# dansolombrino/Kindergarten-VQ-VAE

Measured on AMD Instinct MI355X. Metric: dSentences train sentences/sec, higher is better.
Workload: dtype bf16

## Files before the change

### include/kvq.h

```cpp
#ifndef KVQ_H
#define KVQ_H

#include <stddef.h>
#include <stdint.h>

#ifdef __cplusplus
extern "C" {
#endif

#define KVQ_VERSION 100

#define KVQ_F32 0
#define KVQ_BF16 1

#define KVQ_OK 0
#define KVQ_E_INVALID (-1)
#define KVQ_E_WORKSPACE (-2)
#define KVQ_E_LAUNCH (-3)
#define KVQ_E_NODEVICE (-4)

int kvq_version(void);
const char* kvq_last_error(void);

#define KVQ_GRAPH_NODE_KERNEL 0
// ... 129 lines not shown

size_t kvq_attn_probs_workspace_bytes(int B, int nh, int Sq, int Sk);
int kvq_attn_probs(const void* q, const void* k, const void* v, const int64_t* mask, const float* lse, int B, int nh, int Sq, int Sk,
                   int dh, int ldq, int ldk, int ldv, int causal, float scale, int io_dtype, float* probs, double* table, void* ws,
                   size_t ws_bytes, void* stream);

int kvq_attn_set_variant(int variant);

#define KVQ_GEMM_NT 0
#define KVQ_GEMM_NN 1
#define KVQ_GEMM_TN 2
#define KVQ_GEMM_TILE_128x192 0
#define KVQ_GEMM_TILE_128x256 1
#define KVQ_GEMM_TILE_256x192 2
#define KVQ_GEMM_TILE_256x256 3
#define KVQ_GEMM_TILE_64x128 4
#define KVQ_GEMM_TILE_128x192H 5
#define KVQ_GEMM_PERSISTENT 0x100
typedef struct kvq_gemm_problem {
    const void* A;
    const void* B;
    void* C;
    const void* bias;
    int M, N, K;
    int lda, ldb, ldc;
    int accumulate;
} kvq_gemm_problem;
int kvq_gemm_bf16(const void* A, const void* B, const void* bias, void* C, int M, int N, int K, int lda, int ldb, int ldc,
                  int layout, int tile, int accumulate, void* stream);
int kvq_gemm_any_bf16(const void* A, const void* B, const void* bias, void* C, int M, int N, int K, int lda, int ldb, int ldc,
                      int layout, int accumulate, void* stream);
int kvq_gemm_grouped_bf16(const kvq_gemm_problem* problems, int n_problems, int layout, int tile, void* stream);
int kvq_gemm_grouped_mixed_bf16(const kvq_gemm_problem* problems, const int* tiles, int n_problems, int layout, void* stream);
int kvq_gemm_bf16_dropres(const void* A, const void* B, const void* bias, const void* R, void* C, int M, int N, int K, int lda, int ldb,
                          int ldc, int tile, float p_drop, uint64_t seed, uint32_t site, void* stream);
int kvq_gemm_bf16_gelu(const void* A, const void* B, const void* bias, void* Hout, void* Aout, int M, int N, int K, int lda, int ldb,
                       int ldc, int tile, void* stream);
int64_t kvq_gemm_dgelu_partial_rows(int64_t M, int tile);
int kvq_gemm_bf16_dgelu(const void* A, const void* B, const void* H, void* C, float* part, size_t part_bytes, int M, int N, int K,
                        int lda, int ldb, int ldc, int tile, void* stream);

size_t kvq_gemm_ce_stats_bytes(int M, int N);
int kvq_gemm_bf16_ce(const void* A, const void* B, const void* bias, void* C, int M, int N, int K, int lda, int ldb, int ldc, int V,
                     float* stats, size_t stats_bytes, void* stream);

int kvq_fp8_quantize(const void* x_bf16, int64_t rows, int cols, int64_t ld, void* out_fp8, float* amax, float* scale, void* stream);
int kvq_fp8_state_floats(void);
int kvq_fp8_quantize_delayed(const void* x_bf16, int64_t rows, int cols, int64_t ld, void* out_fp8, float* state, void* stream);
int kvq_fp8_update_scales(float* state, int nsites, float headroom, void* stream);
int kvq_fp8_quantize_segments(const void* src_bf16, const int64_t* seg_off, const int64_t* seg_n, int nseg, int64_t max_seg_n,
                              void* dst_fp8, float* amax, float* scale, void* stream);
int kvq_fp8_quantize_segments_periodic(const void* src_bf16, const int64_t* seg_off, const int64_t* seg_n, int nseg, int64_t max_seg_n,
                                       void* dst_fp8, float* amax, float* scale, const void* step_count_u64, int period, void* stream);
int kvq_gemm_fp8_nt(const void* A8, const void* B8, const float* scale_a, const float* scale_b, const void* bias, void* C, int M, int N,
                    int K, int lda, int ldb, int ldc, void* stream);
int kvq_dropout_residual_ln_fwd_fp8(const void* y, const void* resid, const float* gamma, const float* beta, int64_t N, int H,
                                    float eps, float p_drop, uint64_t seed, uint32_t site, void* out, void* pre, float* mean, float* rstd,
                                    void* out_fp8, float* fp8_state, void* stream);
int kvq_attn_fwd_fp8_ok(int Sq, int Sk);
int kvq_attn_fwd_fp8(const void* q, const void* k, const void* v, const int64_t* mask, int B, int nh, int Sq, int Sk, int dh,
                     int ldq, int ldk, int ldv, int ldo, int causal, float scale, float p_drop, uint64_t seed, uint32_t site,
                     void* out, float* lse, void* out_fp8, int ld8, float* fp8_state, void* stream);
int kvq_gemm_fp8_nt_gelu(const void* A8, const void* B8, const float* scale_a, const float* scale_b, const void* bias, void* Hout, void* Aout,
                         void* Aout_fp8, int ld8, float* fp8_state, int M, int N, int K, int lda, int ldb, int ldc, void* stream);

#define KVQ_FP8_E4M3 0
// ... 99 lines not shown
```

### kindergarten-vq-vae_amd/csrc/kvq_gemm2.hip

```cpp
#include <limits.h>
#include <stdlib.h>

#include <atomic>
#include <type_traits>

#include "kvq_common.h"

namespace kvq {
namespace g2 {

typedef __bf16 bf16x8 __attribute__((ext_vector_type(8)));
typedef short s16x4 __attribute__((ext_vector_type(4)));
typedef __attribute__((address_space(1))) const void* gptr_t;
typedef __attribute__((address_space(3))) void* lptr_t;
typedef __attribute__((address_space(3))) s16x4* l4ptr_t;

constexpr int BK = 64;
constexpr int ROWB = 128;
constexpr int MAX_PROBLEMS = 16;

struct Problem {
    const unsigned short* A;
    const unsigned short* B;
    unsigned short* C;
// ... 1029 lines not shown
    if (P.p[0].M < C::BM || P.p[0].N < C::BN) return fail(KVQ_E_INVALID, "kvq_gemm (persistent): the matrix must hold one whole tile");
    constexpr int LDSP = C::NS * C::STAGE + 2 * BIAS_SLOT;
    static_assert(LDSP <= 160 * 1024, "LDS budget (persistent)");
    static std::atomic<bool> attr_done{false};
    if (!attr_done) {
        hipError_t e = hipFuncSetAttribute(reinterpret_cast<const void*>(&gemm3_kernel<C, EPI>), hipFuncAttributeMaxDynamicSharedMemorySize, LDSP);
        if (e != hipSuccess) return fail(KVQ_E_LAUNCH, "hipFuncSetAttribute(gemm3): %s", hipGetErrorString(e));
        attr_done = true;
    }
    const int grid = P.ntiles < persistent_grid() ? P.ntiles : persistent_grid();
    hipLaunchKernelGGL((gemm3_kernel<C, EPI>), dim3((unsigned)grid), dim3(C::THREADS), LDSP, st, P);
    return check_launch("gemm3_kernel");
}

template <template <bool, bool> class T>
static int launch_layout(int layout, const Params& P, hipStream_t st) {
    switch (layout) {
        case KVQ_GEMM_NT: return launch_cfg<T<true, true>>(P, st);
        case KVQ_GEMM_NN: return launch_cfg<T<true, false>>(P, st);
        case KVQ_GEMM_TN: return launch_cfg<T<false, false>>(P, st);
    }
    return fail(KVQ_E_INVALID, "kvq_gemm_bf16: unknown layout %d", layout);
}

static void tile_of(int tile, int& bm, int& bn) {
    switch (tile) {
        case KVQ_GEMM_TILE_128x256: bm = 128; bn = 256; break;
        case KVQ_GEMM_TILE_256x192: bm = 256; bn = 192; break;
        case KVQ_GEMM_TILE_256x256: bm = 256; bn = 256; break;
        case KVQ_GEMM_TILE_64x128: bm = 64; bn = 128; break;
        case KVQ_GEMM_TILE_128x192H: bm = 128; bn = 192; break;
        default: bm = 128; bn = 192; break;
    }
}

}
}

using namespace kvq;

static int build_params(const kvq_gemm_problem* probs, int nprob, int layout, int tile, g2::Params& P, const char* who) {
    KVQ_REQUIRE(probs && nprob >= 1 && nprob <= g2::MAX_PROBLEMS, "%s: 1..%d problems per launch", who, g2::MAX_PROBLEMS);
    KVQ_REQUIRE(layout == KVQ_GEMM_NT || layout == KVQ_GEMM_NN || layout == KVQ_GEMM_TN, "%s: unknown layout %d", who, layout);
    const bool persistent = (tile & KVQ_GEMM_PERSISTENT) != 0;
    tile &= ~KVQ_GEMM_PERSISTENT;
    KVQ_REQUIRE(tile >= KVQ_GEMM_TILE_128x192 && tile <= KVQ_GEMM_TILE_128x192H, "%s: unknown tile %d", who, tile);
    KVQ_REQUIRE(!(persistent && (tile == KVQ_GEMM_TILE_64x128 || tile == KVQ_GEMM_TILE_128x192H)), "%s: the four-wave tiles have no persistent form", who);
    int bm, bn;
    g2::tile_of(tile, bm, bn);
    (void)persistent;
    P.nprob = nprob;
    int t0 = 0;
    for (int i = 0; i < nprob; ++i) {
        const kvq_gemm_problem& q = probs[i];
        KVQ_REQUIRE(q.A && q.B && q.C && q.M > 0 && q.N > 0 && q.K > 0, "%s: problem %d: bad argument", who, i);
        KVQ_REQUIRE(q.K % g2::BK == 0, "%s: problem %d: K=%d must be a multiple of %d", who, i, q.K, g2::BK);
        KVQ_REQUIRE(q.M % 8 == 0 && q.N % 8 == 0 && q.lda % 8 == 0 && q.ldb % 8 == 0 && q.ldc % 8 == 0 && q.M >= 8 && q.N >= 8,
                    "%s: problem %d: M, N, lda, ldb, ldc must be multiples of 8", who, i);
        KVQ_REQUIRE((((uintptr_t)q.A | (uintptr_t)q.B | (uintptr_t)q.C) & 15) == 0 && (!q.bias || ((uintptr_t)q.bias & 7) == 0),
                    "%s: problem %d: operands must be 16-byte aligned", who, i);
        const int a_cols = layout == KVQ_GEMM_TN ? q.M : q.K, b_cols = layout == KVQ_GEMM_NT ? q.K : q.N;
        KVQ_REQUIRE(q.lda >= a_cols && q.ldb >= b_cols && q.ldc >= q.N, "%s: problem %d: leading dimension too small", who, i);
        g2::Problem& d = P.p[i];
        d.A = (const unsigned short*)q.A; d.B = (const unsigned short*)q.B; d.C = (unsigned short*)q.C; d.bias = (const unsigned short*)q.bias;
        d.M = q.M; d.N = q.N; d.K = q.K; d.lda = q.lda; d.ldb = q.ldb; d.ldc = q.ldc;
        d.tiles_m = (q.M + bm - 1) / bm; d.tiles_n = (q.N + bn - 1) / bn;
// ... 108 lines not shown
    if (nb)
        if (int rc = build_params(sorted, nb, layout, KVQ_GEMM_TILE_256x256, P, who)) return rc;
    const int nbig = P.ntiles;
    if (nprob > nb) {
        if (int rc = build_params(sorted + nb, nprob - nb, layout, KVQ_GEMM_TILE_128x256, S, who)) return rc;
        for (int i = nb; i < nprob; ++i) {
            P.p[i] = S.p[i - nb];
            P.p[i].tile0 += nbig;
        }
        for (int i = nprob; i < g2::MAX_PROBLEMS; ++i) P.p[i] = P.p[0];
        P.ntiles = nbig + S.ntiles;
    }
    P.nprob = nprob;
    typedef g2::Cfg256x256<false, false> CA;
    typedef g2::Cfg128x256<false, false> CB;
    constexpr int LDS = CA::LDS > CB::LDS ? CA::LDS : CB::LDS;
    static std::atomic<bool> attr_done{false};
    if (!attr_done) {
        hipError_t e = hipFuncSetAttribute(reinterpret_cast<const void*>(&g2::gemm2_mixed_kernel<CA, CB>), hipFuncAttributeMaxDynamicSharedMemorySize, LDS);
        if (e != hipSuccess) return fail(KVQ_E_LAUNCH, "hipFuncSetAttribute(gemm2_mixed): %s", hipGetErrorString(e));
        attr_done = true;
    }
    hipLaunchKernelGGL((g2::gemm2_mixed_kernel<CA, CB>), dim3((unsigned)P.ntiles), dim3(CA::THREADS), LDS, (hipStream_t)stream, P, nbig);
    return check_launch("gemm2_mixed_kernel");
}

int kvq_gemm_bf16(const void* A, const void* B, const void* bias, void* C, int M, int N, int K, int lda, int ldb, int ldc,
                  int layout, int tile, int accumulate, void* stream) {
    kvq_gemm_problem q;
    q.A = A; q.B = B; q.C = C; q.bias = bias; q.M = M; q.N = N; q.K = K; q.lda = lda; q.ldb = ldb; q.ldc = ldc; q.accumulate = accumulate;
    return kvq_gemm_grouped_bf16(&q, 1, layout, tile, stream);
}

int kvq_gemm_bf16_gelu(const void* A, const void* B, const void* bias, void* Hout, void* Aout, int M, int N, int K, int lda, int ldb,
                       int ldc, int tile, void* stream) {
    KVQ_REQUIRE(Aout && ((uintptr_t)Aout & 15) == 0, "kvq_gemm_bf16_gelu: null / misaligned second output");
    const int base = tile & ~KVQ_GEMM_PERSISTENT;
    KVQ_REQUIRE(base == KVQ_GEMM_TILE_256x192 || base == KVQ_GEMM_TILE_128x256, "kvq_gemm_bf16_gelu: tile must be 256x192 or 128x256");
    kvq_gemm_problem q;
    q.A = A; q.B = B; q.C = Hout; q.bias = bias; q.M = M; q.N = N; q.K = K; q.lda = lda; q.ldb = ldb; q.ldc = ldc; q.accumulate = 0;
    g2::Params P;
    if (int rc = build_params(&q, 1, KVQ_GEMM_NT, tile, P, "kvq_gemm_bf16_gelu")) return rc;
    for (int i = 0; i < g2::MAX_PROBLEMS; ++i) P.p[i].C2 = (unsigned short*)Aout;
    hipStream_t st = (hipStream_t)stream;
    if (tile & KVQ_GEMM_PERSISTENT) {
        if (base == KVQ_GEMM_TILE_256x192) return g2::launch_persistent<g2::Cfg256x192<true, true>, g2::EPI_GELU>(P, st);
        return g2::launch_persistent<g2::Cfg128x256<true, true>, g2::EPI_GELU>(P, st);
    }
    if (tile == KVQ_GEMM_TILE_256x192) return g2::launch_cfg<g2::Cfg256x192<true, true>, g2::EPI_GELU>(P, st);
    return g2::launch_cfg<g2::Cfg128x256<true, true>, g2::EPI_GELU>(P, st);
}

int kvq_gemm_bf16_dropres(const void* A, const void* B, const void* bias, const void* R, void* C, int M, int N, int K, int lda, int ldb,
                          int ldc, int tile, float p_drop, uint64_t seed, uint32_t site, void* stream) {
    KVQ_REQUIRE(R && ((uintptr_t)R & 15) == 0, "kvq_gemm_bf16_dropres: null / misaligned residual");
    KVQ_REQUIRE(p_drop >= 0.f && p_drop < 1.f, "kvq_gemm_bf16_dropres: p_drop out of range");
    KVQ_REQUIRE(tile == KVQ_GEMM_TILE_128x192 || tile == KVQ_GEMM_TILE_128x256 || tile == KVQ_GEMM_TILE_64x128,
                "kvq_gemm_bf16_dropres: tile must be 128x192, 128x256 or 64x128");
    kvq_gemm_problem q;
    q.A = A; q.B = B; q.C = C; q.bias = bias; q.M = M; q.N = N; q.K = K; q.lda = lda; q.ldb = ldb; q.ldc = ldc; q.accumulate = 0;
    g2::Params P;
    if (int rc = build_params(&q, 1, KVQ_GEMM_NT, tile, P, "kvq_gemm_bf16_dropres")) return rc;
    for (int i = 0; i < g2::MAX_PROBLEMS; ++i) {
        g2::Problem& d = P.p[i];
        d.H = (const unsigned short*)R; d.seed = seed; d.seed_off = seed_offset_ptr(); d.site = site; d.thresh = drop_threshold(p_drop);
        d.inv_keep = p_drop > 0.f ? 1.0f / (1.0f - p_drop) : 1.0f;
// ... 87 lines not shown
```

### kindergarten-vq-vae_amd/kvq/_ffi.py

```python
from __future__ import annotations

import ctypes as C
import os

_PKG = os.path.dirname(os.path.dirname(os.path.abspath(__file__)))
LIB_PATH = os.environ.get("KVQ_LIB_PATH") or os.path.join(_PKG, "lib", "libkvq.so")

KVQ_F32, KVQ_BF16 = 0, 1

_vp, _i64, _int, _f32, _sz = C.c_void_p, C.c_int64, C.c_int, C.c_float, C.c_size_t

KVQ_REDUCE_MAX_ITEMS = 32


class ReduceItem(C.Structure):
    _fields_ = [("src", _vp), ("dst", _vp), ("count", _i64), ("cols", _i64), ("ld", _i64), ("scale", _f32),
                ("src_dtype", C.c_int32), ("dst_dtype", C.c_int32), ("accumulate", C.c_int32)]


class GemmProblem(C.Structure):
    _fields_ = [("A", _vp), ("B", _vp), ("C", _vp), ("bias", _vp), ("M", _int), ("N", _int), ("K", _int),
                ("lda", _int), ("ldb", _int), ("ldc", _int), ("accumulate", _int)]


# ... 37 lines not shown
    "kvq_dropout_residual_ln_fwd": (_int, [_vp, _vp, _vp, _vp, _i64, _int, _f32, _f32, C.c_uint64, C.c_uint32, _int, _vp, _vp, _vp, _vp, _vp]),
    "kvq_ln_bwd_workspace_bytes": (_sz, [_i64, _int]),
    "kvq_dropout_residual_ln_bwd": (_int, [_vp, _vp, _vp, _vp, _vp, _i64, _int, _f32, C.c_uint64, C.c_uint32, _int, _vp, _vp, _vp, _vp, _vp,
                                           _int, _int, _vp, _sz, _vp]),
    "kvq_colsum_workspace_bytes": (_sz, [_i64, _i64]),
    "kvq_colsum": (_int, [_vp, _i64, _i64, _i64, _int, _vp, _int, _f32, _int, _vp, _sz, _vp]),
    "kvq_sum_slabs": (_int, [_vp, _int, _i64, _int, _vp, _vp]),
    "kvq_reduce_batch": (_int, [C.POINTER(ReduceItem), _int, _vp]),
    "kvq_ln_bwd_partial_rows": (_i64, [_i64]),
    "kvq_dropout_residual_ln_bwd_partial": (_int, [_vp, _vp, _vp, _vp, _vp, _i64, _int, _f32, C.c_uint64, C.c_uint32, _int, _vp, _vp,
                                                   _int, _vp, _sz, _vp]),
    "kvq_embed_ln_fwd": (_int, [_vp, _vp, _vp, _vp, _vp, _vp, _i64, _int, _int, _i64, _f32, _f32, C.c_uint64, C.c_uint32, _int, _vp, _vp,
                                _vp, _vp, _vp]),
    "kvq_ln_dropout_bwd_partial": (_int, [_vp, _vp, _vp, _vp, _vp, _i64, _int, _f32, C.c_uint64, C.c_uint32, _int, _vp, _vp, _sz, _vp]),
    "kvq_colsum_partial_rows": (_i64, [_i64]),
    "kvq_colsum_partial": (_int, [_vp, _i64, _i64, _i64, _int, _vp, _sz, _vp]),
    "kvq_gelu_fwd": (_int, [_vp, _vp, _i64, _int, _vp]),
    "kvq_gelu_bwd": (_int, [_vp, _vp, _vp, _i64, _int, _vp]),
    "kvq_gelu_bwd_partial_rows": (_i64, [_i64]),
    "kvq_gelu_bwd_bias": (_int, [_vp, _vp, _vp, _i64, _i64, _int, _vp, _sz, _vp]),
    "kvq_attn_fwd": (_int, [_vp, _vp, _vp, _vp, _int, _int, _int, _int, _int, _int, _int, _int, _int, _int, _f32, _f32,
                            C.c_uint64, C.c_uint32, _int, _vp, _vp, _vp]),
    "kvq_attn_bwd": (_int, [_vp, _vp, _vp, _vp, _vp, _int, _int, _int, _int, _int, _int, _int, _int, _int, _int, _f32, _f32,
                            C.c_uint64, C.c_uint32, _int, _vp, _vp, _vp, _vp, _vp, _vp, _int, _int, _vp]),
    "kvq_attn_bwd_saved": (_int, [_vp, _vp, _vp, _vp, _vp, _vp, _vp, _int, _int, _int, _int, _int, _int, _int, _int, _int, _int, _f32, _f32,
                                  C.c_uint64, C.c_uint32, _int, _vp, _vp, _vp, _vp, _vp, _vp, _int, _int, _vp]),
    "kvq_attn_probs_workspace_bytes": (_sz, [_int, _int, _int, _int]),
    "kvq_attn_probs": (_int, [_vp, _vp, _vp, _vp, _vp, _int, _int, _int, _int, _int, _int, _int, _int, _int, _f32, _int, _vp, _vp, _vp,
                              _sz, _vp]),
    "kvq_gemm_bf16": (_int, [_vp, _vp, _vp, _vp, _int, _int, _int, _int, _int, _int, _int, _int, _int, _vp]),
    "kvq_gemm_any_bf16": (_int, [_vp, _vp, _vp, _vp, _int, _int, _int, _int, _int, _int, _int, _int, _vp]),
    "kvq_gemm_grouped_bf16": (_int, [C.POINTER(GemmProblem), _int, _int, _int, _vp]),
    "kvq_gemm_grouped_mixed_bf16": (_int, [C.POINTER(GemmProblem), C.POINTER(_int), _int, _int, _vp]),
    "kvq_fp8_quantize": (_int, [_vp, _i64, _int, _i64, _vp, _vp, _vp, _vp]),
    "kvq_fp8_state_floats": (_int, []),
    "kvq_fp8_quantize_delayed": (_int, [_vp, _i64, _int, _i64, _vp, _vp, _vp]),
    "kvq_fp8_update_scales": (_int, [_vp, _int, _f32, _vp]),
    "kvq_fp8_quantize_segments": (_int, [_vp, _vp, _vp, _int, _i64, _vp, _vp, _vp, _vp]),
    "kvq_adam_step_dev_fp8": (_int, [_vp, _vp, _vp, _vp, _vp, _vp, _i64, _int, _vp, _f32, _f32, _f32, _f32, _f32, _vp, _vp, _vp, _vp, _vp, _int, _i64, _vp]),
    "kvq_fp8_quantize_segments_periodic": (_int, [_vp, _vp, _vp, _int, _i64, _vp, _vp, _vp, _vp, _int, _vp]),
    "kvq_gemm_fp8_nt": (_int, [_vp, _vp, _vp, _vp, _vp, _vp, _int, _int, _int, _int, _int, _int, _vp]),
    "kvq_gemm_fp8_nt_ex": (_int, [_vp, _vp, _vp, _vp, _vp, _vp, _int, _int, _int, _int, _int, _int, _int, _int, _vp]),
    "kvq_fp8_quantize_fmt": (_int, [_vp, _i64, _int, _i64, _vp, _vp, _vp, _int, _vp]),
    "kvq_fp8_quantize_delayed_fmt": (_int, [_vp, _i64, _int, _i64, _vp, _vp, _int, _vp]),
    "kvq_fp8_update_scales_fmt": (_int, [_vp, _int, _f32, _int, _vp]),
    "kvq_fp8_transpose": (_int, [_vp, _int, _int, _i64, _vp, _i64, _vp]),
    "kvq_fp8_transpose_segments": (_int, [_vp, _vp, _vp, _vp, _vp, _vp, _int, _i64, _vp]),
    "kvq_dropout_residual_ln_fwd_fp8": (_int, [_vp, _vp, _vp, _vp, _i64, _int, _f32, _f32, C.c_uint64, C.c_uint32, _vp, _vp, _vp, _vp, _vp, _vp, _vp]),
    "kvq_attn_fwd_fp8_ok": (_int, [_int, _int]),
    "kvq_attn_fwd_fp8": (_int, [_vp, _vp, _vp, _vp, _int, _int, _int, _int, _int, _int, _int, _int, _int, _int, _f32, _f32,
                                C.c_uint64, C.c_uint32, _vp, _vp, _vp, _int, _vp, _vp]),
    "kvq_gemm_fp8_nt_gelu": (_int, [_vp, _vp, _vp, _vp, _vp, _vp, _vp, _vp, _int, _vp, _int, _int, _int, _int, _int, _int, _vp]),
    "kvq_gemm_bf16_dropres": (_int, [_vp, _vp, _vp, _vp, _vp, _int, _int, _int, _int, _int, _int, _int, _f32, C.c_uint64, C.c_uint32, _vp]),
    "kvq_gemm_bf16_gelu": (_int, [_vp, _vp, _vp, _vp, _vp, _int, _int, _int, _int, _int, _int, _int, _vp]),
    "kvq_gemm_dgelu_partial_rows": (_i64, [_i64, _int]),
    "kvq_gemm_bf16_dgelu": (_int, [_vp, _vp, _vp, _vp, _vp, _sz, _int, _int, _int, _int, _int, _int, _int, _vp]),
    "kvq_attn_set_variant": (_int, [_int]),
    "kvq_adam_step": (_int, [_vp, _vp, _vp, _vp, _vp, _vp, _i64, _int, _f32, _f32, _f32, _f32, _f32, _i64, _f32, _vp]),
    "kvq_ce_forward_stats": (_int, [_vp, _vp, _i64, _i64, _int, _vp, _int, _vp, _vp, _vp, _vp, _vp, _vp]),
    "kvq_ce_forward_stats_ignore": (_int, [_vp, _vp, _i64, _i64, _int, _vp, _int, _i64, _vp, _vp, _vp, _vp, _vp, _vp, _vp]),
    "kvq_gemm_ce_stats_bytes": (_sz, [_int, _int]),
    "kvq_gemm_bf16_ce": (_int, [_vp, _vp, _vp, _vp, _int, _int, _int, _int, _int, _int, _int, _vp, _sz, _vp]),
    "kvq_step_state_advance": (_int, [_vp, _f32, _f32, C.POINTER(_i64), _int, _f32, _f32, _vp]),
    "kvq_adam_step_dev": (_int, [_vp, _vp, _vp, _vp, _vp, _vp, _i64, _int, _vp, _f32, _f32, _f32, _f32, _f32, _vp]),
    "kvq_set_seed_offset": (_int, [_vp]),
    "kvq_grad_sumsq_partials": (_int, []),
# ... 145 lines not shown
```

### kindergarten-vq-vae_amd/kvq/nnops.py

```python
from __future__ import annotations

import torch

from ._ffi import FP8_E4M3, FP8_E5M2, KvqError, check, io_dtype_of, lib, require_gpu, stream_ptr
from .functional import _workspace


def _p(t):
    return None if t is None else t.data_ptr()


def ln_fwd(y, resid, gamma, beta, eps, p_drop=0.0, seed=0, site=0, save_pre=True):
    require_gpu(y, gamma, beta)
    N, H = y.shape
    out = torch.empty_like(y)
    pre = torch.empty_like(y) if save_pre else None
    mean = torch.empty(N, dtype=torch.float32, device=y.device)
    rstd = torch.empty(N, dtype=torch.float32, device=y.device)
    check(lib().kvq_dropout_residual_ln_fwd(y.data_ptr(), _p(resid), gamma.data_ptr(), beta.data_ptr(), N, H, float(eps),
                                            float(p_drop), int(seed), int(site), io_dtype_of(y), out.data_ptr(), _p(pre),
                                            mean.data_ptr(), rstd.data_ptr(), stream_ptr()), "kvq_dropout_residual_ln_fwd")
    return out, pre, mean, rstd


def ln_fwd_fp8(y, resid, gamma, beta, eps, p_drop, seed, site, state, save_pre=True):
    require_gpu(y, gamma, beta)
    N, H = y.shape
    assert y.dtype == torch.bfloat16
    out = torch.empty_like(y)
    out8 = torch.empty((N, H), dtype=torch.uint8, device=y.device)
    pre = torch.empty_like(y) if save_pre else None
    mean = torch.empty(N, dtype=torch.float32, device=y.device)
    rstd = torch.empty(N, dtype=torch.float32, device=y.device)
# ... 455 lines not shown


def dropout(x, p_drop, seed, site, out=None):
    require_gpu(x)
    xc = x.contiguous()
    o = torch.empty_like(xc) if out is None else out
    check(lib().kvq_dropout(xc.data_ptr(), xc.numel(), float(p_drop), int(seed), int(site), io_dtype_of(xc), o.data_ptr(), stream_ptr()),
          "kvq_dropout")
    return o


def zero_ranges(tensors):
    import ctypes
    ts = [t for t in tensors if t is not None]
    if not ts:
        return
    ptrs = (ctypes.c_void_p * len(ts))(*[t.data_ptr() for t in ts])
    sizes = (ctypes.c_int64 * len(ts))(*[t.numel() * t.element_size() for t in ts])
    check(lib().kvq_zero_ranges(ptrs, sizes, len(ts), stream_ptr()), "kvq_zero_ranges")


def embed_grad(g, perm, sorted_ids, gW, accumulate=False):
    require_gpu(g, gW)
    N, H = g.shape
    l = lib()
    ws = _workspace(g.device, l.kvq_embed_grad_workspace_bytes(N, H), tag="embed_grad")
    check(l.kvq_embed_grad(g.data_ptr(), perm.data_ptr(), sorted_ids.data_ptr(), N, H, gW.shape[0], io_dtype_of(g), gW.data_ptr(),
                           io_dtype_of(gW), int(accumulate), ws.data_ptr(), ws.numel(), stream_ptr()), "kvq_embed_grad")
    return gW


_LAYOUTS = {"nt": 0, "nn": 1, "tn": 2}
TILES = {"128x192": 0, "128x256": 1, "256x192": 2, "256x256": 3, "64x128": 4, "128x192h": 5,
         "128x192p": 0x100, "128x256p": 0x101, "256x192p": 0x102, "256x256p": 0x103}
TILE_NAMES = {v: k for k, v in TILES.items()}
_TILE_DIMS = {0: (128, 192), 1: (128, 256), 2: (256, 192), 3: (256, 256), 4: (64, 128)}
def _gemm_dims(a, b, layout):
    if layout == "nt":
        (M, K), N = a.shape, b.shape[0]
    elif layout == "nn":
        (M, K), N = a.shape, b.shape[1]
    else:
        (K, M), N = a.shape, b.shape[1]
    return M, N, K


_TK_ALONE = {0: 0.459, 1: 0.557, 2: 0.891, 3: 1.035, 4: 0.296}
_TK_FULL = {0: 0.825, 1: 0.98, 2: 1.5, 3: 1.83, 4: 0.40}
_TK_PAIR = (0.45, 0.52)
_T_TILE = {0: 1.5, 1: 2.0, 2: 2.5, 3: 3.0, 4: 1.0}


def tile_cost_us(t, M, N, K, n_cu=256):
    bm, bn = _TILE_DIMS[t]
    n = -(-M // bm) * -(-N // bn)
    kt = max(K // 64, 1)
    f = min(n, n_cu) / n_cu
    lerp = lambda a, b: a + (b - a) * f
    w = -(-n // n_cu)
    if t == 4:
        return kt * ((w // 2) * lerp(*_TK_PAIR) + (w % 2) * lerp(_TK_ALONE[t], _TK_FULL[t])) + w * _T_TILE[t]
    return w * (kt * lerp(_TK_ALONE[t], _TK_FULL[t]) + _T_TILE[t])


def pick_tile(M, N, K=768, n_cu=256, candidates=None):
    cand = list(_TILE_DIMS) if candidates is None else [TILES[c] if isinstance(c, str) else c for c in candidates]
    return min(cand, key=lambda t: (tile_cost_us(t, M, N, K, n_cu), -_TILE_DIMS[t][0] * _TILE_DIMS[t][1]))


def persistent_pays(t, M, N, K, layout, accumulate=False, n_cu=256):
    bm, bn = _TILE_DIMS[t]
    if layout != "nt" or accumulate or t == 4 or M < bm or N < bn or K // 64 < 3:
        return False
    per_cu = -(-(-(-M // bm) * -(-N // bn)) // n_cu)
    return 3 <= per_cu <= 12


def cu_count(device):
    return torch.cuda.get_device_properties(device).multi_processor_count


def mixed_split(M, N, n_cu):
    tn = -(-N // 256)
    r = n_cu // tn * 256
    return r if 0 < r < M and -(-(M - r) // 128) * tn <= n_cu else 0

# ... 7 lines not shown


def gemm_problem(a, b, out, layout, bias=None, accumulate=False):
    from ._ffi import GemmProblem
    M, N, K = _gemm_dims(a, b, layout)
    assert a.dtype == torch.bfloat16 and b.dtype == torch.bfloat16 and out.dtype == torch.bfloat16
    assert a.stride(1) == 1 and b.stride(1) == 1 and out.stride(1) == 1 and tuple(out.shape) == (M, N)
    return GemmProblem(a.data_ptr(), b.data_ptr(), out.data_ptr(), _p(bias), M, N, K, a.stride(0), b.stride(0), out.stride(0),
                       int(accumulate))


def pad_rows(t, rows_padded):
    rows, cols = t.shape
    es = t.element_size()
    out = torch.empty((rows_padded, cols), dtype=t.dtype, device=t.device)
    check(lib().kvq_pad_rows(t.data_ptr(), rows, cols * es, t.stride(0) * es, out.data_ptr(), rows_padded, stream_ptr()), "kvq_pad_rows")
    return out


def _pad_ok(t):
    return t.dim() == 2 and t.stride(1) == 1 and (t.shape[1] * t.element_size()) % 16 == 0 and (t.stride(0) * t.element_size()) % 16 == 0 \
        and t.data_ptr() % 16 == 0


def tn_operands_k64(a, b):
    K = a.shape[0]
    if K % 64 == 0 or not (_pad_ok(a) and _pad_ok(b)):
        return None
    Kp = (K + 63) // 64 * 64
    return pad_rows(a, Kp), pad_rows(b, Kp)


_ANY_WARNED = set()
GEMM_ROUTES = {"mfma": 0, "any": 0, "tn_padded": 0, "row_split": 0}


def _warn_any(M, N, K, layout):
    if 2.0 * M * N * K > 64e6 and (M, N, K, layout) not in _ANY_WARNED:
        _ANY_WARNED.add((M, N, K, layout))
        import warnings
        warnings.warn(f"kvq.nnops.gemm: {layout} product M={M} N={N} K={K} ({2e-6 * M * N * K:.0f} MFLOP) runs on the any-shape kernel: "
                      f"the MFMA kernel needs K % 64 == 0, M / N / leading dimensions % 8 == 0 and 16-byte aligned operands", stacklevel=3)


def _gemm_any(a, b, layout, bias, out, accumulate, warn=True):
    M, N, K = _gemm_dims(a, b, layout)
    if a.stride(1) != 1:
        a = a.contiguous()
    if b.stride(1) != 1:
        b = b.contiguous()
    if out.stride(1) != 1 or (bias is not None and bias.stride(0) != 1):
        raise KvqError("kvq.nnops.gemm: output rows / bias must be contiguous")
    if warn:
        _warn_any(M, N, K, layout)
    GEMM_ROUTES["any"] += 1
    check(lib().kvq_gemm_any_bf16(a.data_ptr(), b.data_ptr(), _p(bias), out.data_ptr(), M, N, K, a.stride(0), b.stride(0), out.stride(0),
                                  _LAYOUTS[layout], int(accumulate), stream_ptr()), "kvq_gemm_any_bf16")
    return out


def gemm(a, b, layout="nt", bias=None, out=None, accumulate=False, tile=None):
    require_gpu(a, b)
    M, N, K = _gemm_dims(a, b, layout)
    if a.dtype != torch.bfloat16 or b.dtype != torch.bfloat16 or (out is not None and out.dtype != torch.bfloat16):
        raise KvqError(f"kvq.nnops.gemm: bf16 operands only (got {a.dtype}, {b.dtype})")
    if out is None:
        out = torch.empty((M, N), dtype=a.dtype, device=a.device)
    if not gemm_mfma_ok(a, b, out, layout, bias):
        if layout == "tn" and K % 64 != 0 and K > 64:
            padded = tn_operands_k64(a, b)
            if padded is not None and gemm_mfma_ok(padded[0], padded[1], out, layout, bias):
                GEMM_ROUTES["tn_padded"] += 1
                return gemm(padded[0], padded[1], layout, bias=bias, out=out, accumulate=accumulate, tile=tile)
        if layout != "tn" and M % 8 != 0 and M > 8 and gemm_mfma_ok(a[:M - M % 8], b, out[:M - M % 8], layout, bias):
            M8 = M - M % 8
            GEMM_ROUTES["row_split"] += 1
            gemm(a[:M8], b, layout, bias=bias, out=out[:M8], accumulate=accumulate, tile=tile)
            _gemm_any(a[M8:], b, layout, bias, out[M8:], accumulate, warn=False)
            return out
        return _gemm_any(a, b, layout, bias, out, accumulate)
    if tile == "mixed":
        r = mixed_split(M, N, cu_count(a.device)) if layout == "tn" and bias is None and not accumulate else 0
        if not r:
            raise KvqError(f"kvq.nnops.gemm: tile 'mixed' is for plain tn products that mixed_split() splits (M={M} N={N} {layout})")
        from ._ffi import GemmProblem
        GEMM_ROUTES["mfma"] += 1
        parts = [GemmProblem(a_.data_ptr(), b.data_ptr(), o_.data_ptr(), None, o_.shape[0], N, K, a.stride(0), b.stride(0), out.stride(0), 0)
                 for a_, o_ in ((a[:, :r], out[:r]), (a[:, r:], out[r:]))]
        gemm_grouped_mixed(parts, ["256x256", "128x256"], "tn")
        return out
    if tile is None:
        t = pick_tile(M, N, K)
        if persistent_pays(t, M, N, K, layout, accumulate):
            t |= 0x100
    else:
        t = TILES[tile] if isinstance(tile, str) else tile
    GEMM_ROUTES["mfma"] += 1
    check(lib().kvq_gemm_bf16(a.data_ptr(), b.data_ptr(), _p(bias), out.data_ptr(), M, N, K, a.stride(0), b.stride(0), out.stride(0),
                              _LAYOUTS[layout], t, int(accumulate), stream_ptr()), "kvq_gemm_bf16")
    return out


def gemm_grouped(problems, layout, tile):
    from ._ffi import GemmProblem
    arr = (GemmProblem * len(problems))(*problems)
    t = TILES[tile] if isinstance(tile, str) else tile
    check(lib().kvq_gemm_grouped_bf16(arr, len(problems), _LAYOUTS[layout], t, stream_ptr()), "kvq_gemm_grouped_bf16")


def gemm_grouped_mixed(problems, tiles, layout="tn"):
    import ctypes
    from ._ffi import GemmProblem
    if len(tiles) != len(problems):
        raise KvqError("kvq.nnops.gemm_grouped_mixed: one tile per problem")
    arr = (GemmProblem * len(problems))(*problems)
    ts = (ctypes.c_int * len(tiles))(*[TILES[t] if isinstance(t, str) else t for t in tiles])
    check(lib().kvq_gemm_grouped_mixed_bf16(arr, ts, len(problems), _LAYOUTS[layout], stream_ptr()), "kvq_gemm_grouped_mixed_bf16")


def gemm_gelu(x, w, bias, tile="256x192"):
    M, K = x.shape
    N = w.shape[0]
    h = torch.empty((M, N), dtype=x.dtype, device=x.device)
    a = torch.empty_like(h)
    check(lib().kvq_gemm_bf16_gelu(x.data_ptr(), w.data_ptr(), _p(bias), h.data_ptr(), a.data_ptr(), M, N, K, x.stride(0), w.stride(0),
                                   h.stride(0), TILES[tile], stream_ptr()), "kvq_gemm_bf16_gelu")
    return h, a


DROPRES_TILES = ("128x192", "128x256", "64x128")


# ... 223 lines not shown
```

Baseline: 15210.

## Add stream-K style deep-K split GEMM with fixup kernel for few-tile products

Adds a split-K (stream-K-like) GEMM path that divides tile×k-step units evenly across one workgroup per CU, writes partial fp32 accumulators to a workspace, and runs a fixup kernel that sums partials, adds bias and stores bf16. A cost model routes NN/NT products with fewer 256x256 tiles than CUs to this path by default. It targets under-occupancy when M×N is small but K is deep, at the cost of an extra launch and fp32 workspace traffic.

Result: no change. 15250, median of 6 (+0.3%).

```diff
diff --git a/include/kvq.h b/include/kvq.h
--- a/include/kvq.h
+++ b/include/kvq.h
@@ -185,6 +185,9 @@
                       int layout, int accumulate, void* stream);
 int kvq_gemm_grouped_bf16(const kvq_gemm_problem* problems, int n_problems, int layout, int tile, void* stream);
 int kvq_gemm_grouped_mixed_bf16(const kvq_gemm_problem* problems, const int* tiles, int n_problems, int layout, void* stream);
+size_t kvq_gemm_deepk_workspace_bytes(int M, int N, int workers);
+int kvq_gemm_bf16_deepk(const void* A, const void* B, const void* bias, void* C, int M, int N, int K, int lda, int ldb, int ldc,
+                        int layout, int workers, void* ws, size_t ws_bytes, void* stream);
 int kvq_gemm_bf16_dropres(const void* A, const void* B, const void* bias, const void* R, void* C, int M, int N, int K, int lda, int ldb,
                           int ldc, int tile, float p_drop, uint64_t seed, uint32_t site, void* stream);
 int kvq_gemm_bf16_gelu(const void* A, const void* B, const void* bias, void* Hout, void* Aout, int M, int N, int K, int lda, int ldb,
diff --git a/kindergarten-vq-vae_amd/csrc/kvq_gemm2.hip b/kindergarten-vq-vae_amd/csrc/kvq_gemm2.hip
--- a/kindergarten-vq-vae_amd/csrc/kvq_gemm2.hip
+++ b/kindergarten-vq-vae_amd/csrc/kvq_gemm2.hip
@@ -1085,6 +1085,125 @@
         case KVQ_GEMM_TILE_128x192H: bm = 128; bn = 192; break;
         default: bm = 128; bn = 192; break;
     }
+}
+
+struct DeepK {
+    float* ws;
+    int ntiles, nkt, W, S, g;
+    long long U;
+};
+__device__ __forceinline__ void deepk_tile(const Problem& pr, const DeepK& dk, int t, int& tm, int& tn) {
+    const int r = t % dk.S, j = t / dk.S;
+    band_walk(pr, r * dk.g + j, tm, tn);
+}
+
+template <class C>
+__global__ __launch_bounds__(C::THREADS, C::MINW) void gemm2_deepk_kernel(Problem pr, DeepK dk) {
+    extern __shared__ __attribute__((aligned(16))) char smem[];
+    const int tid = threadIdx.x, lane = tid & 63;
+    const int w = __builtin_amdgcn_readfirstlane(tid >> 6);
+    const int wm = w / C::WN, wn = w % C::WN;
+    const int wk = blockIdx.x;
+    int u = (int)((long long)wk * dk.U / dk.W);
+    const int u1 = (int)((long long)(wk + 1) * dk.U / dk.W);
+    while (u < u1) {
+        const int t = u / dk.nkt, k0 = u - t * dk.nkt;
+        const int n = u1 - u < dk.nkt - k0 ? u1 - u : dk.nkt - k0;
+        int tm, tn;
+        deepk_tile(pr, dk, t, tm, tn);
+        const int m0 = tm * C::BM, n0 = tn * C::BN;
+        f32x4 acc[C::FA][C::FB];
+#pragma unroll
+        for (int mi = 0; mi < C::FA; ++mi)
+#pragma unroll
+            for (int ni = 0; ni < C::FB; ++ni) acc[mi][ni] = 0.f;
+        int la = lane;
+        asm volatile("" : "+v"(la));
+        Stager<C> sg;
+        sg.init(pr, smem, m0, n0, w, la);
+        sg.baseA += (unsigned long long)k0 * sg.stepA;
+        sg.baseB += (unsigned long long)k0 * sg.stepB;
+        constexpr int NPRO = (G2_EARLY_START && C::NS >= 3) ? C::NS - 1 : C::NS;
+#pragma unroll
+        for (int s = 0; s < NPRO; ++s)
+            if (s < n) sg.issue(s);
+        mainloop<C>(acc, sg, smem, n, wm, wn, la);
+        int tb = tid;
+        asm volatile("" : "+v"(tb));
+        if (n == dk.nkt) {
+            u16x4 biasv[C::FB];
+            load_bias<C>(pr, n0, wn, tb & 63, biasv);
+            epilogue<C, EPI_NONE>(pr, smem, acc, biasv, tb, tb & 63, wm, wn, m0, n0, tm, 1.0f);
+        } else {
+            f32x4* slot = reinterpret_cast<f32x4*>(dk.ws) + (size_t)(wk + t) * (size_t)(C::BM * C::BN / 4) + tb;
+#pragma unroll
+            for (int mi = 0; mi < C::FA; ++mi)
+#pragma unroll
+                for (int ni = 0; ni < C::FB; ++ni) slot[(mi * C::FB + ni) * C::THREADS] = acc[mi][ni];
+        }
+        u += n;
+        if (u < u1) {
+            wait_vm<0>();
+            __syncthreads();
+        }
+    }
+}
+
+__device__ __forceinline__ int deepk_owner(const DeepK& dk, long long u) { return (int)(((u + 1) * dk.W - 1) / dk.U); }
+
+template <class C>
+__global__ __launch_bounds__(C::THREADS) void gemm2_deepk_fix_kernel(Problem pr, DeepK dk) {
+    constexpr int ROWS = C::WM * 16, CPR = C::BN / 8;
+    __shared__ __attribute__((aligned(16))) char tile[ROWS * C::CLD];
+    const int tid = threadIdx.x, lane = tid & 63;
+    const int w = __builtin_amdgcn_readfirstlane(tid >> 6);
+    const int wm = w / C::WN, wn = w % C::WN;
+    const int t = blockIdx.x / C::FA, mi = blockIdx.x % C::FA;
+    const int w_lo = deepk_owner(dk, (long long)t * dk.nkt), w_hi = deepk_owner(dk, (long long)(t + 1) * dk.nkt - 1);
+    if (w_lo == w_hi) return;
+    int tm, tn;
+    deepk_tile(pr, dk, t, tm, tn);
+    const int m0 = tm * C::BM, n0 = tn * C::BN;
+    u16x4 biasv[C::FB];
+    load_bias<C>(pr, n0, wn, lane, biasv);
+    f32x4 acc[C::FB];
+#pragma unroll
+    for (int ni = 0; ni < C::FB; ++ni) acc[ni] = 0.f;
+    for (int wk = w_lo; wk <= w_hi; ++wk) {
+        if ((long long)wk * dk.U / dk.W == (long long)(wk + 1) * dk.U / dk.W) continue;
+        const f32x4* slot = reinterpret_cast<const f32x4*>(dk.ws) + (size_t)(wk + t) * (size_t)(C::BM * C::BN / 4) + tid;
+#pragma unroll
+        for (int ni = 0; ni < C::FB; ++ni) acc[ni] = acc[ni] + slot[(mi * C::FB + ni) * C::THREADS];
+    }
+    const int frow = lane & 15, fk = lane >> 4;
+#pragma unroll
+    for (int ni = 0; ni < C::FB; ++ni) {
+        const u16x4 b = biasv[ni];
+        const f32x4 v = acc[ni] + f32x4{bf16_to_f32(b.x), bf16_to_f32(b.y), bf16_to_f32(b.z), bf16_to_f32(b.w)};
+        const u16x4 o = {f32_to_bf16(v.x), f32_to_bf16(v.y), f32_to_bf16(v.z), f32_to_bf16(v.w)};
+        *reinterpret_cast<u16x4*>(tile + (wm * 16 + frow) * C::CLD + (wn * C::TN + ni * 16 + 4 * fk) * 2) = o;
+    }
+    __syncthreads();
+    for (int i = tid; i < ROWS * CPR; i += C::THREADS) {
+        const int r = i / CPR, c16 = i % CPR;
+        const int m = m0 + (r >> 4) * C::TM + mi * 16 + (r & 15), nn = n0 + c16 * 8;
+        if (m < pr.M && nn < pr.N)
+            *reinterpret_cast<uint4*>(pr.C + (size_t)m * pr.ldc + nn) = *reinterpret_cast<const uint4*>(tile + r * C::CLD + c16 * 16);
+    }
+}
+
+template <class C>
+static int launch_deepk(const Params& P, const DeepK& dk, hipStream_t st) {
+    static std::atomic<bool> attr_done{false};
+    if (!attr_done) {
+        hipError_t e = hipFuncSetAttribute(reinterpret_cast<const void*>(&gemm2_deepk_kernel<C>), hipFuncAttributeMaxDynamicSharedMemorySize, C::LDS);
+        if (e != hipSuccess) return fail(KVQ_E_LAUNCH, "hipFuncSetAttribute(gemm2_deepk): %s", hipGetErrorString(e));
+        attr_done = true;
+    }
+    hipLaunchKernelGGL((gemm2_deepk_kernel<C>), dim3((unsigned)dk.W), dim3(C::THREADS), C::LDS, st, P.p[0], dk);
+    if (int rc = check_launch("gemm2_deepk_kernel")) return rc;
+    hipLaunchKernelGGL((gemm2_deepk_fix_kernel<C>), dim3((unsigned)(dk.ntiles * C::FA)), dim3(C::THREADS), 0, st, P.p[0], dk);
+    return check_launch("gemm2_deepk_fix_kernel");
 }
 
 }
@@ -1259,6 +1378,40 @@
     return kvq_gemm_grouped_bf16(&q, 1, layout, tile, stream);
 }
 
+size_t kvq_gemm_deepk_workspace_bytes(int M, int N, int workers) {
+    if (M <= 0 || N <= 0 || workers <= 0) return 0;
+    const size_t ntiles = (size_t)((M + 255) / 256) * (size_t)((N + 255) / 256);
+    return (ntiles + (size_t)workers - 1) * (size_t)(256 * 256 * sizeof(float));
+}
+
+int kvq_gemm_bf16_deepk(const void* A, const void* B, const void* bias, void* C, int M, int N, int K, int lda, int ldb, int ldc,
+                        int layout, int workers, void* ws, size_t ws_bytes, void* stream) {
+    const char* who = "kvq_gemm_bf16_deepk";
+    KVQ_REQUIRE(layout == KVQ_GEMM_NT || layout == KVQ_GEMM_NN, "%s: layout NT or NN", who);
+    KVQ_REQUIRE(workers >= 1 && workers <= 65535, "%s: 1..65535 workers, got %d", who, workers);
+    kvq_gemm_problem q;
+    q.A = A; q.B = B; q.C = C; q.bias = bias; q.M = M; q.N = N; q.K = K; q.lda = lda; q.ldb = ldb; q.ldc = ldc; q.accumulate = 0;
+    g2::Params P;
+    if (int rc = build_params(&q, 1, layout, KVQ_GEMM_TILE_256x256, P, who)) return rc;
+    KVQ_REQUIRE(ws && ((uintptr_t)ws & 15) == 0, "%s: null / misaligned workspace", who);
+    KVQ_REQUIRE(ws_bytes >= kvq_gemm_deepk_workspace_bytes(M, N, workers), "%s: workspace %zu < %zu bytes", who, ws_bytes,
+                kvq_gemm_deepk_workspace_bytes(M, N, workers));
+    g2::DeepK dk;
+    dk.ws = (float*)ws;
+    dk.ntiles = P.ntiles;
+    dk.nkt = K / g2::BK;
+    dk.W = workers;
+    dk.U = (long long)dk.ntiles * dk.nkt;
+    KVQ_REQUIRE(dk.U < (1ll << 30), "%s: %lld units", who, dk.U);
+    int a = dk.W, b = dk.ntiles;
+    while (b) { const int r = a % b; a = b; b = r; }
+    dk.g = a;
+    dk.S = dk.ntiles / dk.g;
+    hipStream_t st = (hipStream_t)stream;
+    if (layout == KVQ_GEMM_NN) return g2::launch_deepk<g2::Cfg256x256<true, false>>(P, dk, st);
+    return g2::launch_deepk<g2::Cfg256x256<true, true>>(P, dk, st);
+}
+
 int kvq_gemm_bf16_gelu(const void* A, const void* B, const void* bias, void* Hout, void* Aout, int M, int N, int K, int lda, int ldb,
                        int ldc, int tile, void* stream) {
     KVQ_REQUIRE(Aout && ((uintptr_t)Aout & 15) == 0, "kvq_gemm_bf16_gelu: null / misaligned second output");
diff --git a/kindergarten-vq-vae_amd/kvq/_ffi.py b/kindergarten-vq-vae_amd/kvq/_ffi.py
--- a/kindergarten-vq-vae_amd/kvq/_ffi.py
+++ b/kindergarten-vq-vae_amd/kvq/_ffi.py
@@ -93,6 +93,8 @@
     "kvq_gemm_any_bf16": (_int, [_vp, _vp, _vp, _vp, _int, _int, _int, _int, _int, _int, _int, _int, _vp]),
     "kvq_gemm_grouped_bf16": (_int, [C.POINTER(GemmProblem), _int, _int, _int, _vp]),
     "kvq_gemm_grouped_mixed_bf16": (_int, [C.POINTER(GemmProblem), C.POINTER(_int), _int, _int, _vp]),
+    "kvq_gemm_deepk_workspace_bytes": (_sz, [_int, _int, _int]),
+    "kvq_gemm_bf16_deepk": (_int, [_vp, _vp, _vp, _vp, _int, _int, _int, _int, _int, _int, _int, _int, _vp, _sz, _vp]),
     "kvq_fp8_quantize": (_int, [_vp, _i64, _int, _i64, _vp, _vp, _vp, _vp]),
     "kvq_fp8_state_floats": (_int, []),
     "kvq_fp8_quantize_delayed": (_int, [_vp, _i64, _int, _i64, _vp, _vp, _vp]),
diff --git a/kindergarten-vq-vae_amd/kvq/nnops.py b/kindergarten-vq-vae_amd/kvq/nnops.py
--- a/kindergarten-vq-vae_amd/kvq/nnops.py
+++ b/kindergarten-vq-vae_amd/kvq/nnops.py
@@ -1,4 +1,6 @@
 from __future__ import annotations
+
+import os
 
 import torch
 
@@ -520,7 +522,8 @@
 
 _LAYOUTS = {"nt": 0, "nn": 1, "tn": 2}
 TILES = {"128x192": 0, "128x256": 1, "256x192": 2, "256x256": 3, "64x128": 4, "128x192h": 5,
-         "128x192p": 0x100, "128x256p": 0x101, "256x192p": 0x102, "256x256p": 0x103}
+         "128x192p": 0x100, "128x256p": 0x101, "256x192p": 0x102, "256x256p": 0x103,
+         "deepk": 0x200}
 TILE_NAMES = {v: k for k, v in TILES.items()}
 _TILE_DIMS = {0: (128, 192), 1: (128, 256), 2: (256, 192), 3: (256, 256), 4: (64, 128)}
 def _gemm_dims(a, b, layout):
@@ -539,7 +542,36 @@
 _T_TILE = {0: 1.5, 1: 2.0, 2: 2.5, 3: 3.0, 4: 1.0}
 
 
+DEEPK = 0x200
+_TK_DEEP = 1.445
+_T_DEEP = 36.0
+_T_FIX = 2.0
+_FIX_BYTES_PER_US = 5.5e6
+_DEEP_REF = 0.85
+
+
+def deepk_cost_us(M, N, K, n_cu=256):
+    tiles = -(-M // 256) * -(-N // 256)
+    units = tiles * max(K // 64, 1)
+    per = -(-units // n_cu)
+    f = min(units, n_cu) / n_cu
+    pieces = min(tiles + n_cu - 1, units) if units > tiles else 0
+    return per * (_TK_ALONE[3] + (_TK_DEEP - _TK_ALONE[3]) * f) + _T_DEEP + _T_FIX + pieces * 256 * 256 * 4 / _FIX_BYTES_PER_US
+
+
+def deepk_enabled():
+    return os.environ.get("KVQ_DEEPK", "1") != "0"
+
+
+def deepk_pays(t, M, N, K, layout, accumulate=False, n_cu=256):
+    if layout not in ("nn", "nt") or accumulate or -(-M // 256) * -(-N // 256) >= n_cu:
+        return False
+    return tile_cost_us(DEEPK, M, N, K, n_cu) < _DEEP_REF * tile_cost_us(t & 0xff, M, N, K, n_cu)
+
+
 def tile_cost_us(t, M, N, K, n_cu=256):
+    if t == DEEPK:
+        return deepk_cost_us(M, N, K, n_cu)
     bm, bn = _TILE_DIMS[t]
     n = -(-M // bm) * -(-N // bn)
     kt = max(K // 64, 1)
@@ -613,7 +645,7 @@
 
 
 _ANY_WARNED = set()
-GEMM_ROUTES = {"mfma": 0, "any": 0, "tn_padded": 0, "row_split": 0}
+GEMM_ROUTES = {"mfma": 0, "any": 0, "tn_padded": 0, "row_split": 0, "deepk": 0}
 
 
 def _warn_any(M, N, K, layout):
@@ -672,13 +704,34 @@
         return out
     if tile is None:
         t = pick_tile(M, N, K)
-        if persistent_pays(t, M, N, K, layout, accumulate):
+        if deepk_enabled() and deepk_pays(t, M, N, K, layout, accumulate, cu_count(a.device)):
+            t = DEEPK
+        elif persistent_pays(t, M, N, K, layout, accumulate):
             t |= 0x100
     else:
         t = TILES[tile] if isinstance(tile, str) else tile
+    if t == DEEPK:
+        return gemm_deepk(a, b, layout, bias=bias, out=out, accumulate=accumulate)
     GEMM_ROUTES["mfma"] += 1
     check(lib().kvq_gemm_bf16(a.data_ptr(), b.data_ptr(), _p(bias), out.data_ptr(), M, N, K, a.stride(0), b.stride(0), out.stride(0),
                               _LAYOUTS[layout], t, int(accumulate), stream_ptr()), "kvq_gemm_bf16")
+    return out
+
+
+def gemm_deepk(a, b, layout, bias=None, out=None, accumulate=False, workers=None):
+    require_gpu(a, b)
+    M, N, K = _gemm_dims(a, b, layout)
+    if out is None:
+        out = torch.empty((M, N), dtype=a.dtype, device=a.device)
+    if layout not in ("nn", "nt") or accumulate or not gemm_mfma_ok(a, b, out, layout, bias):
+        raise KvqError(f"kvq.nnops.gemm: tile 'deepk' is for plain nn / nt products the MFMA kernel takes (M={M} N={N} K={K} {layout})")
+    W = cu_count(a.device) if workers is None else int(workers)
+    l = lib()
+    ws = _workspace(a.device, l.kvq_gemm_deepk_workspace_bytes(M, N, W), tag=("gemm_deepk", torch.cuda.current_stream(a.device).cuda_stream))
+    GEMM_ROUTES["mfma"] += 1
+    GEMM_ROUTES["deepk"] += 1
+    check(l.kvq_gemm_bf16_deepk(a.data_ptr(), b.data_ptr(), _p(bias), out.data_ptr(), M, N, K, a.stride(0), b.stride(0), out.stride(0),
+                                _LAYOUTS[layout], W, ws.data_ptr(), ws.numel(), stream_ptr()), "kvq_gemm_bf16_deepk")
     return out
 
 
```
